# Gregor-Mendel-Institute/SNPmatch

Measured on AMD Instinct MI355X. Metric: accession×SNP comparisons/sec (whole node); achieved HBM GB/s vs peak, higher is better.
Workload: dtype f64

## Files before the change

include/snpmatch_hip.h:

```cpp
#ifndef SNPMATCH_HIP_H
#define SNPMATCH_HIP_H

#include <stdint.h>

#ifdef __cplusplus
extern "C" {
#endif

#define SNPM_OK            0
#define SNPM_ERR_BADARG   -1
#define SNPM_ERR_HIP      -2
#define SNPM_ERR_OOM      -3
#define SNPM_ERR_STATE    -4
#define SNPM_ERR_DOMAIN   -5
#define SNPM_ERR_RCCL     -6

#define SNPM_MODE_EXACT   0
#define SNPM_MODE_STRICT  1
#define SNPM_MODE_FAST    2

typedef struct snpm_ctx   snpm_ctx;
typedef struct snpm_panel snpm_panel;
typedef struct snpm_query snpm_query;
typedef struct snpm_carry snpm_carry;
// ... 108 lines not shown

int snpm_score_dense_host(snpm_ctx *ctx, const int8_t *db, int64_t db_pitch, int64_t n, int64_t n_acc,
                          const double *wei, int skip_hets, double *score, int64_t *ninfo);

int snpm_likelihood(snpm_ctx *ctx, const double *y, const int64_t *n, int64_t m, int64_t len,
                    int truncate, double amin_or_nan, double *lik, double *lrt);
int snpm_likelihood_device(snpm_ctx *ctx, const void *d_y, const void *d_n, int64_t m, int64_t len,
                           int truncate, double amin_or_nan, void *d_lik, void *d_lrt, int *domain_error);

int snpm_binom_identity(snpm_ctx *ctx, const double *x, const int64_t *n, int64_t len, double error_rate,
                        double pthres, int64_t *out, double *sf);
int snpm_binom_sf_host(const double *k, const double *n, int64_t len, double p, double *sf);

int snpm_intersect_sorted(const int64_t *a, int64_t na, const int64_t *b, int64_t nb, int64_t *ia, int64_t *ib,
                          int64_t *n_out);
int snpm_intersect_sorted_search(const int64_t *a, int64_t na, const int64_t *b, int64_t nb, int64_t *ia, int64_t *ib,
                                 int64_t *n_out);
int snpm_panel_segregating(snpm_panel *panel, const int32_t *cols, int64_t ncols, uint8_t *mask);
int snpm_panel_segregating_first(snpm_panel *panel, const int32_t *cols, int64_t ncols, uint8_t *mask, uint8_t *first);
int snpm_query_gather_columns(snpm_query *query, const int32_t *acc_idx, int ncols, uint8_t *codes);
int snpm_query_f1_pairs(snpm_query *query, const int32_t *acc_idx, int n_sel, double *score, int64_t *ninfo);

int snpm_debug_stream_read(snpm_panel *panel, int64_t *bytes_read);
int snpm_profile_enable(snpm_ctx *ctx, int on);
int snpm_profile_reset(snpm_ctx *ctx);
int snpm_profile_read(snpm_ctx *ctx, const char *kernel, int64_t *launches, double *total_ms);

typedef struct snpm_vcf snpm_vcf;
int snpm_vcf_parse(const char *path, int sample_index, snpm_vcf **out);
int snpm_vcf_dims(const snpm_vcf *vcf, int64_t *n_records, int *chr_width, int *gt_width, int *flags, int *n_samples);
int snpm_vcf_fill(const snpm_vcf *vcf, char *chr, int64_t *pos, char *gt, double *pl, int64_t *dp);
int snpm_vcf_fill_u32(const snpm_vcf *vcf, uint32_t *chr, int64_t *pos, uint32_t *gt, double *pl, int64_t *dp, uint8_t *called);
const char *snpm_vcf_sample_name(const snpm_vcf *vcf, int i);
int snpm_vcf_free(snpm_vcf *vcf);

typedef struct snpm_h5 snpm_h5;
int snpm_h5_open(const char *path, snpm_h5 **out);
int snpm_h5_close(snpm_h5 *file);
const char *snpm_h5_last_error(const snpm_h5 *file);
int snpm_h5_list(snpm_h5 *file, const char *group, char *buf, int64_t cap, int64_t *needed);
int snpm_h5_info(snpm_h5 *file, const char *path, const char *attr, int *kind, int *rank, int64_t *dims, int *type_class,
                 int *elem_size, int *is_signed, int64_t *chunk, int *n_attrs);
int snpm_h5_attr_name(snpm_h5 *file, const char *path, int index, char *buf, int64_t cap);
int snpm_h5_read(snpm_h5 *file, const char *path, const char *attr, void *out, int64_t out_bytes);
int snpm_h5_read_rows(snpm_h5 *file, const char *path, const int64_t *row_idx, int64_t file_row0, int64_t nrows, int64_t col0,
                      int64_t ncols, void *out, int64_t out_pitch);
// ... 8 lines not shown
```

snpmatch_amd/_lib.py:

```python
import ctypes as C
import os
import sys

import numpy as np

_HERE = os.path.dirname(os.path.abspath(__file__))
LIB_PATH = os.environ.get("SNPMATCH_HIP_LIB") or os.path.join(_HERE, "libsnpmatch_hip.so")

SNPM_OK = 0
SNPM_ERR_BADARG = -1
SNPM_ERR_HIP = -2
SNPM_ERR_OOM = -3
SNPM_ERR_STATE = -4
SNPM_ERR_DOMAIN = -5
SNPM_ERR_RCCL = -6
GROUP_ID_BYTES = 128
GROUP_LOOPBACK = 1

MODE_EXACT = 0
MODE_STRICT = 1
MODE_FAST = 2

SYMBOLS = [
    "snpm_version", "snpm_hip_build_version", "snpm_build_id", "snpm_device_count", "snpm_init", "snpm_destroy", "snpm_last_error", "snpm_set_stream",
    "snpm_synchronize", "snpm_device_mem_info", "snpm_panel_create", "snpm_panel_create_packed", "snpm_panel_is_packed", "snpm_panel_set_total_accessions", "snpm_panel_row_pitch", "snpm_panel_free", "snpm_panel_info", "snpm_panel_upload_rows", "snpm_panel_load_file", "snpm_panel_load_file_rows", "snpm_panel_load_file_rows_packed", "snpm_pack_rows_host",
    "snpm_panel_upload_wait", "snpm_panel_download_rows", "snpm_panel_fill_synthetic", "snpm_query_create",
    "snpm_query_free", "snpm_query_bind_outputs", "snpm_query_run", "snpm_query_run_device", "snpm_query_error_bound",
    "snpm_query_run_windows", "snpm_query_run_windows_carry", "snpm_score_dense_host", "snpm_likelihood", "snpm_likelihood_device",
    "snpm_binom_identity", "snpm_binom_sf_host", "snpm_intersect_sorted", "snpm_panel_segregating",
    "snpm_query_f1_pairs", "snpm_intersect_sorted_search",
    "snpm_vcf_parse", "snpm_vcf_dims", "snpm_vcf_fill", "snpm_vcf_fill_u32", "snpm_vcf_sample_name", "snpm_vcf_free",
    "snpm_debug_stream_read", "snpm_profile_enable", "snpm_profile_reset", "snpm_profile_read",
    "snpm_panel_fill_synthetic_rows", "snpm_sample_synthetic", "snpm_query_create_device", "snpm_query_last_reeval",
    "snpm_query_last_kernel", "snpm_carry_create", "snpm_carry_reset", "snpm_carry_free", "snpm_carry_set_columns", "snpm_carry_bind_outputs", "snpm_panel_segregating_first", "snpm_query_gather_columns", "snpm_query_run_windows_fast", "snpm_score_batch", "snpm_score_batch_coded", "snpm_batch_configure", "snpm_batch_last_stats", "snpm_genotype_once", "snpm_genotype_once_coded", "snpm_host_alloc", "snpm_host_free",
    "snpm_query_run_carry", "snpm_carry_finish", "snpm_carry_patch", "snpm_carry_device_ptrs", "snpm_carry_error_bound",
    "snpm_group_unique_id", "snpm_group_create_rank", "snpm_group_create_local", "snpm_group_free", "snpm_group_last_error",
    "snpm_group_info", "snpm_group_ctx", "snpm_group_shard", "snpm_group_gather_scores", "snpm_group_gathered_ptrs",
    "snpm_group_transport",
    "snpm_h5_open", "snpm_h5_close", "snpm_h5_last_error", "snpm_h5_list", "snpm_h5_info", "snpm_h5_attr_name", "snpm_h5_read",
    "snpm_h5_read_rows", "snpm_panel_load_h5",
]

_lib = None


class SnpmError(RuntimeError):
    def __init__(self, code, msg):
        RuntimeError.__init__(self, "libsnpmatch_hip error %d: %s" % (code, msg))
        self.code = code
        self.msg = msg


HIP_RUNTIME = "system"


# ... 136 lines not shown
    lib.snpm_host_free.argtypes = [p, p]
    lib.snpm_score_batch.argtypes = [p, i64, p, p, p, ci, i64, ci, ci, p, p, p, p, p]
    lib.snpm_batch_configure.argtypes = [p, ci, ci, dbl]
    lib.snpm_batch_last_stats.argtypes = [p, p]
    lib.snpm_score_dense_host.argtypes = [p, p, i64, i64, i64, p, ci, p, p]
    lib.snpm_likelihood.argtypes = [p, p, p, i64, i64, ci, dbl, p, p]
    lib.snpm_likelihood_device.argtypes = [p, p, p, i64, i64, ci, dbl, p, p, C.POINTER(ci)]
    lib.snpm_binom_identity.argtypes = [p, p, p, i64, dbl, dbl, p, p]
    lib.snpm_binom_sf_host.argtypes = [p, p, i64, dbl, p]
    lib.snpm_intersect_sorted.argtypes = [p, i64, p, i64, p, p, C.POINTER(i64)]
    lib.snpm_panel_segregating.argtypes = [p, p, i64, p]
    lib.snpm_query_f1_pairs.argtypes = [p, p, ci, p, p]
    lib.snpm_panel_segregating_first.argtypes = [p, p, i64, p, p]
    lib.snpm_query_gather_columns.argtypes = [p, p, ci, p]
    lib.snpm_intersect_sorted_search.argtypes = [p, i64, p, i64, p, p, C.POINTER(i64)]
    lib.snpm_vcf_parse.argtypes = [C.c_char_p, ci, pp]
    lib.snpm_vcf_dims.argtypes = [p, C.POINTER(i64), C.POINTER(ci), C.POINTER(ci), C.POINTER(ci), C.POINTER(ci)]
    lib.snpm_vcf_fill.argtypes = [p, p, p, p, p, p]
    lib.snpm_vcf_fill_u32.argtypes = [p, p, p, p, p, p, p]
    lib.snpm_vcf_sample_name.argtypes = [p, ci]
    lib.snpm_vcf_sample_name.restype = C.c_char_p
    lib.snpm_vcf_free.argtypes = [p]
    lib.snpm_debug_stream_read.argtypes = [p, C.POINTER(i64)]
    lib.snpm_profile_enable.argtypes = [p, ci]
    lib.snpm_profile_reset.argtypes = [p]
    lib.snpm_profile_read.argtypes = [p, C.c_char_p, C.POINTER(i64), C.POINTER(dbl)]
    for name in SYMBOLS:
        getattr(lib, name)
    _lib = lib
    return lib


def build_id():
    return load().snpm_build_id().decode()


def check_group(rc, group_handle=None):
    if rc == SNPM_OK:
        return
    msg = load().snpm_group_last_error(group_handle)
    msg = msg.decode("utf-8", "replace") if msg else ""
    if rc == SNPM_ERR_BADARG:
        raise AssertionError(msg)
    if rc == SNPM_ERR_DOMAIN:
        raise AssertionError(msg or "provided y is greater than n")
    if rc == SNPM_ERR_OOM:
# ... 99 lines not shown
```

snpmatch_amd/csrc/snpm_api_launch.hpp:

```cpp
struct FastGeom {
    int bpl, wpb;
    int tile_rows = TILE_ROWS;
    int64_t n_wc, n_colblocks, n_parts, part_rows;
    int64_t n_epochs, n_slots, n_groups;
};

template <int BPL, bool SKIP, bool GATHER, bool NT>
int occupancy_of(int threads)
{
    int nb = 0;
    if (hipOccupancyMaxActiveBlocksPerMultiprocessor(&nb, k_fast<BPL, SKIP, GATHER, NT>, threads, 0) != hipSuccess) nb = 0;
    return nb;
}

int pick_bpl(snpm_ctx *ctx, int64_t n_acc)
{
    (void)n_acc;
    if (ctx->force_bpl == 8 || ctx->force_bpl == 16) return ctx->force_bpl;
    return 4;
}

FastGeom fast_geom(snpm_ctx *ctx, int64_t n_acc, int64_t n, int occ_blocks_hint, int bpl, int tile_rows = TILE_ROWS,
                   int wpb_fixed = 0, int kernel_parts_mult = 1)
{
// ... 41 lines not shown
    n_parts = std::min(n_parts, n_tiles);
    if (ctx->debug_max_parts > 0) n_parts = std::min<int64_t>(n_parts, ctx->debug_max_parts);
    n_parts = std::min<int64_t>(n_parts, 65535);
    g.n_parts = n_parts;
    const int64_t tiles_per_part = (n_tiles + n_parts - 1) / n_parts;
    g.part_rows = tiles_per_part * tile_rows;
    g.n_epochs = std::max<int64_t>(1, (tiles_per_part + EPOCH_TILES - 1) / EPOCH_TILES);
    g.n_slots = g.n_epochs * g.n_parts;
    g.n_groups = (g.n_slots + REDUCE_GROUP - 1) / REDUCE_GROUP;
    return g;
}

template <int BPL, bool SKIP, bool GATHER, bool NT>
int launch_fast_t(snpm_query *q, const FastGeom &g)
{
    snpm_ctx *ctx = q->panel->ctx;
    snpm_panel *p = q->panel;
    dim3 grid((unsigned)g.n_colblocks, (unsigned)g.n_parts);
    dim3 block(WAVE * g.wpb);
    ProfScope ps(ctx, PK_FAST);
    if (BPL == 4 && g.tile_rows == LONG_TILE_ROWS)
        hipLaunchKernelGGL((k_fast<BPL, SKIP, GATHER, NT, false, (BPL == 4 ? LONG_TILE_ROWS : TILE_ROWS)>), grid, block, 0, ctx->stream, p->d,
                           p->pitch, q->d_row_idx, q->row0, q->n, q->d_lut, (double *)ctx->ws_part_score.p, (uint32_t *)ctx->ws_part_miss.p,
                           p->ld, (const int64_t *)nullptr);
    else
        hipLaunchKernelGGL((k_fast<BPL, SKIP, GATHER, NT>), grid, block, 0, ctx->stream, p->d, p->pitch, q->d_row_idx, q->row0,
                           q->n, q->d_lut, (double *)ctx->ws_part_score.p, (uint32_t *)ctx->ws_part_miss.p, p->ld,
                           (const int64_t *)nullptr, (BPL == 4 && g.tile_rows < TILE_ROWS) ? g.tile_rows : 0);
    HIPCHK(ctx, hipGetLastError());
    return SNPM_OK;
}

template <int BPL, bool NT>
int launch_fast_b(snpm_query *q, const FastGeom &g, bool skip, bool gather)
{
    if (skip)
        return gather ? launch_fast_t<BPL, true, true, NT>(q, g) : launch_fast_t<BPL, true, false, NT>(q, g);
    return gather ? launch_fast_t<BPL, false, true, NT>(q, g) : launch_fast_t<BPL, false, false, NT>(q, g);
}

static int q4_waves_per_block(int64_t n_acc)
{
    const int64_t n_wc = (n_acc + 1023) / 1024;
    if (n_wc <= 8) return (int)n_wc;
    int best = 4;
    int64_t best_waves = (n_wc + 3) / 4 * 4;
    for (int w : {7, 8}) {
        const int64_t waves = (n_wc + w - 1) / w * w;
        if (waves <= best_waves) {
            best = w;
// ... 99 lines not shown
```

snpmatch_amd/csrc/snpm_api_oneshot.hpp:

```cpp
int snpm_score_dense_host(snpm_ctx *ctx, const int8_t *db, int64_t db_pitch, int64_t n, int64_t n_acc,
                          const double *wei, int skip_hets, double *score, int64_t *ninfo)
{
    if (!ctx) return SNPM_ERR_BADARG;
    CHECK_ARG(ctx, n >= 0 && n_acc >= 1, "please provide same number of positions for both sample and db");
    CHECK_ARG(ctx, n == 0 || (db != nullptr && wei != nullptr), "NULL input");
    CHECK_ARG(ctx, db_pitch >= n_acc, "db_pitch smaller than n_acc");
    snpm_panel *p = nullptr;
    snpm_query *q = nullptr;
    int rc = snpm_panel_create(ctx, n, n_acc, &p);
    if (rc) return rc;
    rc = snpm_panel_upload_rows(p, 0, n, db, db_pitch);
    if (!rc) rc = snpm_query_create(p, nullptr, 0, n, wei, &q);
    if (!rc) {
        rc = snpm_query_run(q, std::max<int64_t>(n, 1), skip_hets, SNPM_MODE_STRICT, score, ninfo, nullptr);
    }
    std::string keep = ctx->err;
    if (q) snpm_query_free(q);
    (void)snpm_panel_upload_wait(p);
    snpm_panel_free(p);
    if (rc) ctx->err = keep;
    return rc;
}

int snpm_likelihood_device(snpm_ctx *ctx, const void *d_y, const void *d_n, int64_t m, int64_t len, int truncate,
// ... 232 lines not shown
    HIPCHK(ctx, hipStreamSynchronize(st));
    return SNPM_OK;
} SNPM_GUARD(((q && q->panel) ? q->panel->ctx : nullptr))

int snpm_debug_stream_read(snpm_panel *p, int64_t *bytes_read)
{
    CHECK_PANEL(p);
    snpm_ctx *ctx = p->ctx;
    HIPCHK(ctx, hipSetDevice(ctx->device));
    int rc = ensure(ctx, ctx->ws_flags, sizeof(int));
    if (rc) return rc;
    rc = wait_upload(p);
    if (rc) return rc;
    const int64_t n_dwords = p->n_snp * p->pitch / 4;
    const unsigned blocks = (unsigned)std::max<int64_t>(1, std::min<int64_t>((n_dwords + 1023) / 1024, (int64_t)ctx->n_cu * 8));
    hipLaunchKernelGGL(k_calib_read, dim3(blocks), dim3(256), 0, ctx->stream, (const uint32_t *)p->d, n_dwords,
                       (uint32_t *)ctx->ws_flags.p);
    HIPCHK(ctx, hipGetLastError());
    HIPCHK(ctx, hipStreamSynchronize(ctx->stream));
    if (bytes_read) *bytes_read = n_dwords * 4;
    return SNPM_OK;
}

int snpm_host_alloc(snpm_ctx *ctx, int64_t bytes, void **out)
{
    if (!ctx) return SNPM_ERR_BADARG;
    CHECK_ARG(ctx, out != nullptr && bytes >= 0, "bad arguments");
    HIPCHK(ctx, hipSetDevice(ctx->device));
    *out = nullptr;
    hipError_t e = hipHostMalloc(out, (size_t)std::max<int64_t>(bytes, 1), hipHostMallocDefault);
    if (e != hipSuccess) return set_err(ctx, SNPM_ERR_OOM, "hipHostMalloc of %lld bytes failed: %s", (long long)bytes, hipGetErrorString(e));
    return SNPM_OK;
}

int snpm_host_free(snpm_ctx *ctx, void *ptr)
{
    if (!ctx) return SNPM_ERR_BADARG;
    if (ptr && hip_alive()) {
        (void)hipSetDevice(ctx->device);
        (void)hipStreamSynchronize(ctx->copy_stream);
        (void)hipStreamSynchronize(ctx->stream);
        (void)hipHostFree(ptr);
    }
    return SNPM_OK;
}

// ... 1 lines not shown
```

snpmatch_amd/csrc/snpm_api_seg.hpp:

```cpp
struct SegJob {
    snpm_panel *p = nullptr;
    const int64_t *d_row_idx = nullptr;
    int64_t row0 = 0, n_total = 0;
    const double *d_w = nullptr, *d_lut = nullptr;
    const int64_t *seg_off = nullptr;
    int64_t n_seg = 0;
    int64_t chunk = 1000;
    int skip = 0;
    bool certify = true;
    double *d_score = nullptr;
    int64_t *d_ninfo = nullptr;
    int64_t ldo = 0;
    int64_t kmax = 1;
    int cap = 0;
    const int64_t *d_seg_off = nullptr;
};

constexpr int SEG_PAIR_CAP = 32768;

int *seg_pair_count(snpm_ctx *ctx) { return (int *)ctx->ws_pairs.p; }
int32_t *seg_pairs(snpm_ctx *ctx) { return (int32_t *)((char *)ctx->ws_pairs.p + 16); }

template <bool NT>
static int launch_q4_seg(snpm_ctx *ctx, const SegJob &j, dim3 grid, dim3 block, int64_t n_parts, const int64_t *d_desc)
// ... 10 lines not shown
        if (tr == 16) LAUNCH_SEG_TR(S, G, 16);                                                                    \
        else if (tr == 32) LAUNCH_SEG_TR(S, G, 32);                                                               \
        else LAUNCH_SEG_TR(S, G, 64);                                                                             \
    } while (0)
    if (j.skip) {
        if (gather) LAUNCH_SEG(true, true); else LAUNCH_SEG(true, false);
    } else {
        if (gather) LAUNCH_SEG(false, true); else LAUNCH_SEG(false, false);
    }
#undef LAUNCH_SEG_TR
#undef LAUNCH_SEG
    HIPCHK(ctx, hipGetLastError());
    return SNPM_OK;
}

template <int BPL, bool NT>
static int launch_fast_seg(snpm_ctx *ctx, const SegJob &j, dim3 grid, dim3 block, int64_t n_parts, const int64_t *d_desc)
{
    snpm_panel *p = j.p;
    const bool gather = j.d_row_idx != nullptr;
    ProfScope ps(ctx, PK_FAST);
#define LAUNCH_SEG(S, G)                                                                                          \
    hipLaunchKernelGGL((k_fast<BPL, S, G, NT, true>), grid, block, 0, ctx->stream, p->d, p->pitch, j.d_row_idx, j.row0,    \
                       n_parts, j.d_lut, (double *)ctx->ws_part_score.p, (uint32_t *)ctx->ws_part_miss.p, p->ld, d_desc)
    if (j.skip) {
        if (gather) LAUNCH_SEG(true, true); else LAUNCH_SEG(true, false);
    } else {
        if (gather) LAUNCH_SEG(false, true); else LAUNCH_SEG(false, false);
    }
#undef LAUNCH_SEG
    HIPCHK(ctx, hipGetLastError());
    return SNPM_OK;
}

struct SegPlan {
    FastGeom g0;
    int64_t n_parts = 0, tiles_per_part = 0;
    std::vector<int64_t> slot0;
    const int64_t *d_slot0 = nullptr, *d_desc = nullptr;
};

static int seg_plan(snpm_ctx *ctx, SegJob &j, SegPlan &pl)
{
    snpm_panel *p = j.p;
    const int64_t n_seg = j.n_seg;
    const bool q4 = p->packed != 0;
    pl.g0 = q4 ? fast_geom(ctx, p->n_acc, TILE_ROWS, 2, 16, TILE_ROWS, q4_waves_per_block(p->n_acc))
// ... 289 lines not shown
```

snpmatch_amd/csrc/snpm_api_strict.hpp:

```cpp
static inline bool single_accession(const snpm_panel *p) { return p->n_acc_total == 1; }

static int launch_strict_single(snpm_ctx *ctx, const snpm_panel *p, const int64_t *d_row_idx, int64_t row0, const double *d_w,
                                int skip, const int64_t *seg_off, int64_t chunk, int64_t n, int64_t seg0, int64_t n_seg,
                                const int32_t *pairs, const int *count, int cap, int tier, int64_t kmax, dim3 grid,
                                double *out_score, uint32_t *out_miss, int64_t ld)
{
    const bool gather = d_row_idx != nullptr;
#define LAUNCH_SINGLE(S, G)                                                                                          \
    hipLaunchKernelGGL((k_strict_single<S, G>), grid, dim3(SINGLE_THREADS), 0, ctx->stream, p->d, p->kpitch, p->desc,  \
                       d_row_idx, row0, d_w, seg_off, chunk, n, seg0, n_seg, pairs, count, cap, tier, kmax, out_score,  \
                       out_miss, ld)
    if (skip) {
        if (gather) LAUNCH_SINGLE(true, true); else LAUNCH_SINGLE(true, false);
    } else {
        if (gather) LAUNCH_SINGLE(false, true); else LAUNCH_SINGLE(false, false);
    }
#undef LAUNCH_SINGLE
    HIPCHK(ctx, hipGetLastError());
    return SNPM_OK;
}

int launch_strict_dense(snpm_query *q, int skip, const int64_t *d_seg_off, int64_t chunk, int64_t seg0, int64_t n_seg,
                        const int *gate)
{
// ... 113 lines not shown
        dim3 sgrid((unsigned)std::min<int64_t>((total + 255) / 256, (int64_t)ctx->n_cu * 8));
        const bool use_T = !q->transient_panel && q->n >= ctx->acc_major_min_rows && p->dT_state == 1;
        ProfScope ps(ctx, PK_STRICT);
        if (single_accession(p)) {
            q->reeval_path = 2;
            rc = launch_strict_single(ctx, p, q->d_row_idx, q->row0, q->d_w, skip, d_seg_off, chunk, q->n, 0, n_seg, nullptr, d_ncols,
                                      REEVAL_CAP, 1, 0, dim3((unsigned)std::min<int64_t>(n_seg, 65535)),
                                      (double *)ctx->ws_seg_score.p, (uint32_t *)ctx->ws_seg_miss.p, ld);
            if (rc) return rc;
        } else if (use_T) {
            q->reeval_path = 1;
#define LAUNCH_SPARSE_T(S, G)                                                                                      \
    hipLaunchKernelGGL((k_strict_sparse_T<S, G>), sgrid, dim3(256), 0, ctx->stream, p->dT, p->pitchT, q->d_row_idx, \
                       q->row0, q->d_w, d_seg_off, chunk, q->n, n_seg, d_cols, d_ncols, REEVAL_CAP, \
                       (double *)ctx->ws_seg_score.p, (uint32_t *)ctx->ws_seg_miss.p, ld)
            if (skip) {
                if (gather) LAUNCH_SPARSE_T(true, true); else LAUNCH_SPARSE_T(true, false);
            } else {
                if (gather) LAUNCH_SPARSE_T(false, true); else LAUNCH_SPARSE_T(false, false);
            }
#undef LAUNCH_SPARSE_T
        } else {
            q->reeval_path = 2;
#define LAUNCH_SPARSE(S, G)                                                                                        \
    hipLaunchKernelGGL((k_strict_sparse<S, G>), sgrid, dim3(256), 0, ctx->stream, p->d, p->kpitch, p->desc, q->d_row_idx, \
                       q->row0, q->d_w, d_seg_off, chunk, q->n, n_seg, d_cols, d_ncols, REEVAL_CAP, \
                       (double *)ctx->ws_seg_score.p, (uint32_t *)ctx->ws_seg_miss.p, ld)
            if (skip) {
                if (gather) LAUNCH_SPARSE(true, true); else LAUNCH_SPARSE(true, false);
            } else {
                if (gather) LAUNCH_SPARSE(false, true); else LAUNCH_SPARSE(false, false);
            }
#undef LAUNCH_SPARSE
        }
        HIPCHK(ctx, hipGetLastError());
    }
    ProfScope ps(ctx, PK_SCAN);
    if (tail)
        hipLaunchKernelGGL(k_once_tail, dim3(1), dim3(256), 0, ctx->stream, (const double *)ctx->ws_seg_score.p, n_seg, ld, d_ncols,
                           REEVAL_CAP, (double *)ctx->ws_tmp_score.p, d_cols, patch_score, tail->d_ninfo, tail->n_acc, tail->want_lik,
                           tail->state, tail->lik_tmp, tail->out);
    else
        hipLaunchKernelGGL(k_scan_few, dim3(1), dim3(256), 0, ctx->stream, (const double *)ctx->ws_seg_score.p, n_seg, ld,
                           d_ncols, REEVAL_CAP, (double *)ctx->ws_tmp_score.p, carry, d_cols, patch_score);
    HIPCHK(ctx, hipGetLastError());
    return SNPM_OK;
}

// ... 1 lines not shown
```

snpmatch_amd/csrc/snpm_k_fast.hpp:

```cpp
#pragma once

namespace snpm {
typedef uint32_t u32x2 __attribute__((ext_vector_type(2)));
typedef uint32_t u32x4 __attribute__((ext_vector_type(4)));

template <int BPL>
struct LoadT;
template <>
struct LoadT<4> { typedef uint32_t type; };
template <>
struct LoadT<8> { typedef u32x2 type; };
template <>
struct LoadT<16> { typedef u32x4 type; };

__device__ __forceinline__ uint32_t dword_of(const uint32_t &v, int) { return v; }
__device__ __forceinline__ uint32_t dword_of(const u32x2 &v, int k) { return k == 0 ? v.x : v.y; }
__device__ __forceinline__ uint32_t dword_of(const u32x4 &v, int k)
{
    return k == 0 ? v.x : (k == 1 ? v.y : (k == 2 ? v.z : v.w));
}

template <int NDW, bool SKIP, int U>
__device__ __forceinline__ void fast_row(const uint32_t (&x)[NDW], uint32_t group_base, uint32_t roff4,
                                         double (&acc)[NDW * 4], uint32_t (&miss8)[NDW])
// ... 22 lines not shown
#pragma unroll
    for (int e = 0; e < NDW * 4; ++e) acc[e] += w[e];
}

template <int BPL, bool NT>
__device__ __forceinline__ void load_row(const int8_t *p, uint32_t (&x)[BPL / 4])
{
    typedef typename LoadT<BPL>::type load_t;
    load_t v;
    if (NT)
        v = __builtin_nontemporal_load(reinterpret_cast<const load_t *>(p));
    else
        v = *reinterpret_cast<const load_t *>(p);
#pragma unroll
    for (int k = 0; k < BPL / 4; ++k) x[k] = dword_of(v, k);
}

#define SCORE_ROW(U, X, GROUP_BASE, ROFF4, ROFF) fast_row<NDW, SKIP, U>((X), (GROUP_BASE), (ROFF4), acc, miss8)

template <int BPL, bool SKIP, bool GATHER, bool NT, bool SEG = false, int TR = TILE_ROWS>
__global__ void __launch_bounds__(WAVE *MAX_WAVES_PER_BLOCK, (BPL <= 4 ? SNPM_FAST_MIN_WAVES : 1))
k_fast(const int8_t *__restrict__ db, int64_t pitch, const int64_t *__restrict__ row_idx, int64_t row0, int64_t n,
       const double *__restrict__ lut, double *__restrict__ out_score, uint32_t *__restrict__ out_miss, int64_t ld,
       const int64_t *__restrict__ part_desc = nullptr, int tile_rows_rt = 0)
{
    static_assert(BPL == 4 || BPL == 8 || BPL == 16, "int8 panels: 4, 8 or 16 bytes per lane");
    constexpr int NDW = BPL / 4;
    constexpr int EPL = BPL;
    constexpr int G = GATHER ? SNPM_FAST_G_GATHER : SNPM_FAST_G;
    __shared__ __attribute__((aligned(256))) double s_lut[2][TR * 4];
    const int TRR = (tile_rows_rt > 0 && tile_rows_rt <= TR) ? tile_rows_rt : TR;

    const int tid = threadIdx.x;
    const int nthr = blockDim.x;
    const int64_t byte0 = ((int64_t)blockIdx.x * nthr + tid) * BPL;
    const int64_t col0 = byte0;
    const bool lane_on = byte0 < pitch && col0 < ld;
    const int64_t p = SEG ? (int64_t)blockIdx.y + (int64_t)gridDim.y * blockIdx.z : (int64_t)blockIdx.y;
    if (SEG && p >= n) return;
    const int64_t rbase = SEG ? part_desc[3 * p] : 0;
    const int64_t rend = SEG ? part_desc[3 * p + 1] : n;
    const int64_t P = SEG ? 1 : (int64_t)gridDim.y;
    const int64_t T0 = SEG ? 0 : p;
    const int64_t slot0 = SEG ? part_desc[3 * p + 2] : p;
    const int64_t slot_stride = SEG ? 1 : (int64_t)gridDim.y;
    const int64_t n_tiles_total = (rend - rbase + TRR - 1) / TRR;

    double acc[EPL];
    uint32_t miss16[NDW * 2];
    uint32_t miss8[NDW];
#pragma unroll
    for (int i = 0; i < EPL; ++i) acc[i] = 0.0;
#pragma unroll
    for (int i = 0; i < NDW * 2; ++i) miss16[i] = 0;
#pragma unroll
    for (int i = 0; i < NDW; ++i) miss8[i] = 0;

    const uint32_t lane_off = lane_on ? (uint32_t)byte0 : 0u;
    auto row_ptr = [&](int64_t rr) -> const int8_t * {
        const int64_t prow = GATHER ? row_idx[rr] : (row0 + rr);
        const int8_t *rowbase = db + prow * pitch;
        uint32_t off = lane_off;
        asm volatile("" : "+v"(off));
        return rowbase + off;
    };

    auto store_partials = [&](int64_t epoch) {
        if (lane_on) {
            double *os = out_score + (slot0 + epoch * slot_stride) * ld + col0;
            uint32_t *om = out_miss + (slot0 + epoch * slot_stride) * ld + col0;
#pragma unroll
            for (int i = 0; i < EPL; i += 2) *reinterpret_cast<double2 *>(os + i) = make_double2(acc[i], acc[i + 1]);
#pragma unroll
            for (int k = 0; k < NDW; ++k) {
                uint4 m;
                m.x = miss16[2 * k + 0] & 0xffffu;
                m.y = miss16[2 * k + 1] & 0xffffu;
                m.z = miss16[2 * k + 0] >> 16;
                m.w = miss16[2 * k + 1] >> 16;
                *reinterpret_cast<uint4 *>(om + 4 * k) = m;
            }
// ... 114 lines not shown
```

snpmatch_amd/csrc/snpm_k_io.hpp:

```cpp
#pragma once

namespace snpm {
__global__ void k_pack_rows(const int8_t *__restrict__ src, int64_t src_pitch, int64_t nrows, int64_t n_acc,
                            uint8_t *__restrict__ db, int64_t pitch, int64_t desc, int64_t row0, int *__restrict__ bad)
{
    const int64_t row_bytes = pitch + pk_tail_pitch(desc);
    const int64_t i = (int64_t)blockIdx.x * blockDim.x + threadIdx.x;
    if (i >= nrows * row_bytes) return;
    const int64_t r = i / row_bytes, b = i - r * row_bytes;
    uint32_t out = 0;
    int saw = 0;
#pragma unroll
    for (int f = 0; f < 4; ++f) {
        const int64_t a = b * 4 + f;
        int v = -1;
        if (a < n_acc) v = src[r * src_pitch + a];
        saw |= (v > 2);
        out |= (uint32_t)(v < 0 ? 3 : (v & 3)) << (2 * f);
    }
    if (saw) atomicOr(bad, 1);
    db[pk_off(pitch, desc, row0 + r, b)] = (uint8_t)out;
}

__global__ void k_repitch_canon(const int8_t *__restrict__ src, int64_t src_pitch, int64_t nrows, int64_t n_acc,
// ... 121 lines not shown
    }
    wei[3 * r] = w[0];
    wei[3 * r + 1] = w[1];
    wei[3 * r + 2] = w[2];
}

__global__ void __launch_bounds__(256)
k_calib_read(const uint32_t *__restrict__ p, int64_t n_dwords, uint32_t *__restrict__ out)
{
    int64_t i = (int64_t)blockIdx.x * blockDim.x + threadIdx.x;
    const int64_t stride = (int64_t)gridDim.x * blockDim.x;
    uint32_t acc = 0;
    for (; i + 3 * stride < n_dwords; i += 4 * stride) {
        const uint32_t a = __builtin_nontemporal_load(p + i);
        const uint32_t b = __builtin_nontemporal_load(p + i + stride);
        const uint32_t c = __builtin_nontemporal_load(p + i + 2 * stride);
        const uint32_t d = __builtin_nontemporal_load(p + i + 3 * stride);
        acc ^= a ^ b ^ c ^ d;
    }
    for (; i < n_dwords; i += stride) acc ^= __builtin_nontemporal_load(p + i);
    if (acc == 0x9e3779b9u) out[0] = acc;
}

}
```

snpmatch_amd/csrc/snpm_k_strict.hpp:

```cpp
#pragma once

namespace snpm {
template <bool SKIP, bool GATHER>
__global__ void __launch_bounds__(256)
k_strict(const int8_t *__restrict__ db, int64_t pitch, int64_t packed, const int64_t *__restrict__ row_idx, int64_t row0,
         const double *__restrict__ w, const int64_t *__restrict__ seg_off, int64_t chunk, int64_t n, int64_t seg0,
         int64_t n_seg, const int32_t *__restrict__ cols, int64_t ncols, double *__restrict__ out_score,
         uint32_t *__restrict__ out_miss, int64_t ld, const int *__restrict__ gate, int gate_cap)
{
    if (dense_tier_off(gate, gate_cap)) return;
    const int64_t i = (int64_t)blockIdx.y * blockDim.x + threadIdx.x;
    if (i >= ncols) return;
    const int64_t col = cols ? (int64_t)cols[i] : i;
    for (int64_t seg = blockIdx.x; seg < n_seg; seg += gridDim.x) {
    int64_t r0, r1;
    seg_bounds(seg_off, chunk, n, seg_off ? seg : seg0 + seg, r0, r1);
    double a_ref = 0.0, a_het = 0.0, a_alt = 0.0;
    uint32_t miss = 0;
    int64_t r = r0;
    for (; r + 4 <= r1; r += 4) {
        int b[4];
#pragma unroll
        for (int u = 0; u < 4; ++u) {
            const int64_t prow = GATHER ? row_idx[r + u] : (row0 + r + u);
// ... 265 lines not shown
        const int64_t tp = pk_tail_pitch(desc);
        const int64_t byte0 = (int64_t)blockIdx.y * blockDim.x;
        if (tp && byte0 >= pitch) {
            strict4_segments<SKIP, GATHER, true, true>(db + pk_tail_off(desc), tp, row_idx, row0, w, seg_off, chunk, n, seg0, n_seg, ncols,
                                                       out_score, out_miss, ld, c0, s_lut, (uint32_t)pitch);
            return;
        }
        strict4_segments<SKIP, GATHER, true, true>(db, pitch, row_idx, row0, w, seg_off, chunk, n, seg0, n_seg, ncols,
                                                   out_score, out_miss, ld, c0, s_lut);
        return;
    }
    if (c0 >= ncols) return;
    if constexpr (!PACKED && SNPM_STRICT_EXEC) {
        if (*other_codes == 0) {
            strict4_segments<SKIP, GATHER, false, true>(db, pitch, row_idx, row0, w, seg_off, chunk, n, seg0, n_seg, ncols,
                                                        out_score, out_miss, ld, c0, nullptr);
            return;
        }
    }
    strict4_segments<SKIP, GATHER, PACKED, false>(db, pitch, row_idx, row0, w, seg_off, chunk, n, seg0, n_seg, ncols,
                                                  out_score, out_miss, ld, c0, nullptr);
}

template <bool SKIP, bool GATHER>
__global__ void __launch_bounds__(256)
k_strict_sparse(const int8_t *__restrict__ db, int64_t pitch, int64_t packed, const int64_t *__restrict__ row_idx,
                int64_t row0, const double *__restrict__ w, const int64_t *__restrict__ seg_off, int64_t chunk, int64_t n,
                int64_t n_seg, const int32_t *__restrict__ cols, const int *__restrict__ d_ncols, int cap,
                double *__restrict__ out_score, uint32_t *__restrict__ out_miss, int64_t ld)
{
    const int64_t ncols = *d_ncols;
    if (ncols > cap) return;
    for (int64_t id = (int64_t)blockIdx.x * blockDim.x + threadIdx.x; id < n_seg * ncols; id += (int64_t)gridDim.x * blockDim.x) {
    const int64_t seg = id / ncols;
    const int64_t i = id - seg * ncols;
    const int64_t col = cols[i];
    int64_t r0, r1;
    seg_bounds(seg_off, chunk, n, seg, r0, r1);
    double a_ref = 0.0, a_het = 0.0, a_alt = 0.0;
    uint32_t miss = 0;
    constexpr int U = 32;
    int64_t r = r0;
    for (; r + U <= r1; r += U) {
        int b[U];
#pragma unroll
        for (int u = 0; u < U; ++u) {
            const int64_t prow = GATHER ? row_idx[r + u] : (row0 + r + u);
            b[u] = code_at(db, pitch, prow, col, packed);
        }
#pragma unroll
        for (int u = 0; u < U; ++u) {
            const double w0 = w[3 * (r + u) + 0], w1 = w[3 * (r + u) + 1], w2 = w[3 * (r + u) + 2];
            a_ref = add_sel(a_ref, b[u] == 0, w0);
            if (!SKIP) a_het = add_sel(a_het, b[u] == 2, w1);
            a_alt = add_sel(a_alt, b[u] == 1, w2);
            miss += SKIP ? (b[u] < 0 || b[u] == 2) : (b[u] < 0);
        }
    }
    for (; r < r1; ++r) {
        const int64_t prow = GATHER ? row_idx[r] : (row0 + r);
        const int b = code_at(db, pitch, prow, col, packed);
        const double w0 = w[3 * r + 0], w1 = w[3 * r + 1], w2 = w[3 * r + 2];
        a_ref = add_sel(a_ref, b == 0, w0);
        if (!SKIP) a_het = add_sel(a_het, b == 2, w1);
        a_alt = add_sel(a_alt, b == 1, w2);
        miss += SKIP ? (b < 0 || b == 2) : (b < 0);
    }
    out_score[seg * ld + i] = ((0.0 + a_ref) + a_het) + a_alt;
    out_miss[seg * ld + i] = miss;
    }
}

constexpr int PT_ROWS = 256;
constexpr int PT_COLS = 64;
__global__ void __launch_bounds__(256)
k_pack_transpose(const int8_t *__restrict__ db, int64_t pitch, int64_t n_snp, int64_t n_acc,
                 uint8_t *__restrict__ dT, int64_t pitchT, int *__restrict__ bad)
{
    __shared__ uint32_t tile[PT_ROWS][PT_COLS / 4 + 1];
    const int64_t snp0 = (int64_t)blockIdx.x * PT_ROWS;
    const int64_t acc0 = (int64_t)blockIdx.y * PT_COLS;
    const int t = threadIdx.x;
    for (int pass = 0; pass < PT_ROWS / 16; ++pass) {
        const int r = pass * 16 + (t >> 4);
        const int64_t row = snp0 + r;
        uint32_t v = 0xffffffffu;
        if (row < n_snp) v = *reinterpret_cast<const uint32_t *>(db + row * pitch + acc0 + (t & 15) * 4);
        tile[r][t & 15] = v;
    }
    __syncthreads();
    const int c = t & 63, q = t >> 6;
    if (acc0 + c < n_acc) {
// ... 268 lines not shown
```

snpmatch_amd/engine.py:

```python
import atexit
import ctypes as C
import weakref

import numpy as np

from . import _lib
from ._lib import MODE_EXACT, MODE_FAST, MODE_STRICT, check, ptr

_default_ctx = None


class Context(object):
    def __init__(self, device_id=0, _borrowed=None):
        lib = _lib.load()
        if _borrowed is None:
            h = C.c_void_p()
            rc = lib.snpm_init(int(device_id), C.byref(h))
            check(rc, None)
        else:
            h = _borrowed
        self._owns = _borrowed is None
        self.lib = lib
        self.h = h
        self.device_id = int(device_id)
# ... 372 lines not shown

    def fill_synthetic(self, seed, snp0=0, acc0=0, row0=0, nrows=None):
        nrows = self.n_snp - row0 if nrows is None else nrows
        check(self.ctx.lib.snpm_panel_fill_synthetic_rows(self.h, C.c_uint64(int(seed)), int(snp0), int(acc0), int(row0),
                                                          int(nrows)), self.ctx.h)

    def segregating_rows(self, cols):
        cols = np.ascontiguousarray(cols, dtype=np.int32)
        mask = np.zeros(self.n_snp, dtype=np.uint8)
        check(self.ctx.lib.snpm_panel_segregating(self.h, ptr(cols), len(cols), ptr(mask)), self.ctx.h)
        return mask

    def segregating_first(self, cols):
        cols = np.ascontiguousarray(cols, dtype=np.int32)
        mask = np.zeros(self.n_snp, dtype=np.uint8)
        first = np.full(self.n_snp, 0xFF, dtype=np.uint8)
        check(self.ctx.lib.snpm_panel_segregating_first(self.h, ptr(cols), len(cols), ptr(mask), ptr(first)), self.ctx.h)
        return mask, first

    def stream_read(self):
        n = C.c_int64(0)
        check(self.ctx.lib.snpm_debug_stream_read(self.h, C.byref(n)), self.ctx.h)
        return n.value

    def free(self):
        if self.h:
            for q in list(self._queries):
                q.free()
            if self.ctx.h:
                self.ctx.lib.snpm_panel_free(self.h)
            self.h = None

    def __del__(self):
        try:
            self.free()
        except Exception:
            pass


class Query(object):

    def __init__(self, panel, row_idx, wei, row0=0, _device=None):
        self.panel = panel
        ctx = panel.ctx
        if _device is not None:
            d_rows, d_wei, n = _device
# ... 749 lines not shown
```

Measured before the change: 6173 billion.

## Warp-specialize sparse strict reeval with double-buffered LDS tiles and add touch probe

Rewrites k_strict_sparse so that one wave computes while three loader waves prefetch the column codes of the next row tile into a double-buffered shared-memory tile. Several segments are packed into each wave by lane, and the grid is capped at a multiple of the CU count. The aim is to hide the latency of scattered per-column gathers, at the cost of idle lanes when ncols does not divide WAVE and an early exit when ncols exceeds WAVE. Separately, k_fast now checks lane validity against n_acc and clamps inactive lanes to a valid offset, and a debug column-touch timing probe is added.

```diff
diff --git a/include/snpmatch_hip.h b/include/snpmatch_hip.h
--- a/include/snpmatch_hip.h
+++ b/include/snpmatch_hip.h
@@ -154,6 +154,7 @@
 int snpm_query_f1_pairs(snpm_query *query, const int32_t *acc_idx, int n_sel, double *score, int64_t *ninfo);
 
 int snpm_debug_stream_read(snpm_panel *panel, int64_t *bytes_read);
+int snpm_debug_touch_columns(snpm_panel *panel, const int32_t *cols, int k, double *ms, int64_t *touches);
 int snpm_profile_enable(snpm_ctx *ctx, int on);
 int snpm_profile_reset(snpm_ctx *ctx);
 int snpm_profile_read(snpm_ctx *ctx, const char *kernel, int64_t *launches, double *total_ms);
diff --git a/snpmatch_amd/_lib.py b/snpmatch_amd/_lib.py
--- a/snpmatch_amd/_lib.py
+++ b/snpmatch_amd/_lib.py
@@ -30,7 +30,7 @@
     "snpm_binom_identity", "snpm_binom_sf_host", "snpm_intersect_sorted", "snpm_panel_segregating",
     "snpm_query_f1_pairs", "snpm_intersect_sorted_search",
     "snpm_vcf_parse", "snpm_vcf_dims", "snpm_vcf_fill", "snpm_vcf_fill_u32", "snpm_vcf_sample_name", "snpm_vcf_free",
-    "snpm_debug_stream_read", "snpm_profile_enable", "snpm_profile_reset", "snpm_profile_read",
+    "snpm_debug_stream_read", "snpm_debug_touch_columns", "snpm_profile_enable", "snpm_profile_reset", "snpm_profile_read",
     "snpm_panel_fill_synthetic_rows", "snpm_sample_synthetic", "snpm_query_create_device", "snpm_query_last_reeval",
     "snpm_query_last_kernel", "snpm_carry_create", "snpm_carry_reset", "snpm_carry_free", "snpm_carry_set_columns", "snpm_carry_bind_outputs", "snpm_panel_segregating_first", "snpm_query_gather_columns", "snpm_query_run_windows_fast", "snpm_score_batch", "snpm_score_batch_coded", "snpm_batch_configure", "snpm_batch_last_stats", "snpm_genotype_once", "snpm_genotype_once_coded", "snpm_host_alloc", "snpm_host_free",
     "snpm_query_run_carry", "snpm_carry_finish", "snpm_carry_patch", "snpm_carry_device_ptrs", "snpm_carry_error_bound",
@@ -213,6 +213,7 @@
     lib.snpm_vcf_sample_name.restype = C.c_char_p
     lib.snpm_vcf_free.argtypes = [p]
     lib.snpm_debug_stream_read.argtypes = [p, C.POINTER(i64)]
+    lib.snpm_debug_touch_columns.argtypes = [p, C.POINTER(C.c_int32), C.c_int, C.POINTER(C.c_double), C.POINTER(i64)]
     lib.snpm_profile_enable.argtypes = [p, ci]
     lib.snpm_profile_reset.argtypes = [p]
     lib.snpm_profile_read.argtypes = [p, C.c_char_p, C.POINTER(i64), C.POINTER(dbl)]
diff --git a/snpmatch_amd/csrc/snpm_api_launch.hpp b/snpmatch_amd/csrc/snpm_api_launch.hpp
--- a/snpmatch_amd/csrc/snpm_api_launch.hpp
+++ b/snpmatch_amd/csrc/snpm_api_launch.hpp
@@ -87,10 +87,10 @@
     if (BPL == 4 && g.tile_rows == LONG_TILE_ROWS)
         hipLaunchKernelGGL((k_fast<BPL, SKIP, GATHER, NT, false, (BPL == 4 ? LONG_TILE_ROWS : TILE_ROWS)>), grid, block, 0, ctx->stream, p->d,
                            p->pitch, q->d_row_idx, q->row0, q->n, q->d_lut, (double *)ctx->ws_part_score.p, (uint32_t *)ctx->ws_part_miss.p,
-                           p->ld, (const int64_t *)nullptr);
+                           p->ld, p->n_acc, (const int64_t *)nullptr);
     else
         hipLaunchKernelGGL((k_fast<BPL, SKIP, GATHER, NT>), grid, block, 0, ctx->stream, p->d, p->pitch, q->d_row_idx, q->row0,
-                           q->n, q->d_lut, (double *)ctx->ws_part_score.p, (uint32_t *)ctx->ws_part_miss.p, p->ld,
+                           q->n, q->d_lut, (double *)ctx->ws_part_score.p, (uint32_t *)ctx->ws_part_miss.p, p->ld, p->n_acc,
                            (const int64_t *)nullptr, (BPL == 4 && g.tile_rows < TILE_ROWS) ? g.tile_rows : 0);
     HIPCHK(ctx, hipGetLastError());
     return SNPM_OK;
diff --git a/snpmatch_amd/csrc/snpm_api_oneshot.hpp b/snpmatch_amd/csrc/snpm_api_oneshot.hpp
--- a/snpmatch_amd/csrc/snpm_api_oneshot.hpp
+++ b/snpmatch_amd/csrc/snpm_api_oneshot.hpp
@@ -278,6 +278,44 @@
     return SNPM_OK;
 }
 
+int snpm_debug_touch_columns(snpm_panel *p, const int32_t *cols, int k, double *ms, int64_t *touches)
+{
+    CHECK_PANEL(p);
+    snpm_ctx *ctx = p->ctx;
+    CHECK_ARG(ctx, !p->packed, "the touch probe reads int8 panels");
+    CHECK_ARG(ctx, cols != nullptr && k >= 1 && k <= 1024, "cols: 1..1024 accession columns");
+    for (int j = 0; j < k; ++j) CHECK_ARG(ctx, cols[j] >= 0 && cols[j] < p->n_acc, "column out of range");
+    HIPCHK(ctx, hipSetDevice(ctx->device));
+    int rc = ensure(ctx, ctx->ws_flags, sizeof(int));
+    if (rc) return rc;
+    rc = wait_upload(p);
+    if (rc) return rc;
+    int32_t *d_cols = nullptr;
+    HIPCHK(ctx, hipMalloc(&d_cols, (size_t)k * sizeof(int32_t)));
+    hipEvent_t e0 = nullptr, e1 = nullptr;
+    hipError_t err = hipMemcpyAsync(d_cols, cols, (size_t)k * sizeof(int32_t), hipMemcpyHostToDevice, ctx->stream);
+    if (err == hipSuccess) err = hipEventCreate(&e0);
+    if (err == hipSuccess) err = hipEventCreate(&e1);
+    const unsigned blocks = (unsigned)ctx->n_cu * 8;
+    for (int it = 0; it < 2 && err == hipSuccess; ++it) {
+        if (it == 1) err = hipEventRecord(e0, ctx->stream);
+        hipLaunchKernelGGL(k_touch_cols, dim3(blocks), dim3(256), 0, ctx->stream, p->d, p->pitch, p->n_snp, d_cols, k,
+                           (uint32_t *)ctx->ws_flags.p);
+        if (err == hipSuccess) err = hipGetLastError();
+    }
+    if (err == hipSuccess) err = hipEventRecord(e1, ctx->stream);
+    if (err == hipSuccess) err = hipEventSynchronize(e1);
+    float t = 0.0f;
+    if (err == hipSuccess) err = hipEventElapsedTime(&t, e0, e1);
+    if (e0) (void)hipEventDestroy(e0);
+    if (e1) (void)hipEventDestroy(e1);
+    (void)hipFree(d_cols);
+    HIPCHK(ctx, err);
+    if (ms) *ms = t;
+    if (touches) *touches = p->n_snp * (int64_t)k;
+    return SNPM_OK;
+}
+
 int snpm_host_alloc(snpm_ctx *ctx, int64_t bytes, void **out)
 {
     if (!ctx) return SNPM_ERR_BADARG;
diff --git a/snpmatch_amd/csrc/snpm_api_seg.hpp b/snpmatch_amd/csrc/snpm_api_seg.hpp
--- a/snpmatch_amd/csrc/snpm_api_seg.hpp
+++ b/snpmatch_amd/csrc/snpm_api_seg.hpp
@@ -56,7 +56,7 @@
     ProfScope ps(ctx, PK_FAST);
 #define LAUNCH_SEG(S, G)                                                                                          \
     hipLaunchKernelGGL((k_fast<BPL, S, G, NT, true>), grid, block, 0, ctx->stream, p->d, p->pitch, j.d_row_idx, j.row0,    \
-                       n_parts, j.d_lut, (double *)ctx->ws_part_score.p, (uint32_t *)ctx->ws_part_miss.p, p->ld, d_desc)
+                       n_parts, j.d_lut, (double *)ctx->ws_part_score.p, (uint32_t *)ctx->ws_part_miss.p, p->ld, p->n_acc, d_desc)
     if (j.skip) {
         if (gather) LAUNCH_SEG(true, true); else LAUNCH_SEG(true, false);
     } else {
diff --git a/snpmatch_amd/csrc/snpm_api_strict.hpp b/snpmatch_amd/csrc/snpm_api_strict.hpp
--- a/snpmatch_amd/csrc/snpm_api_strict.hpp
+++ b/snpmatch_amd/csrc/snpm_api_strict.hpp
@@ -159,8 +159,9 @@
 #undef LAUNCH_SPARSE_T
         } else {
             q->reeval_path = 2;
+            const dim3 rgrid((unsigned)std::min<int64_t>(n_seg, (int64_t)ctx->n_cu * 6));
 #define LAUNCH_SPARSE(S, G)                                                                                        \
-    hipLaunchKernelGGL((k_strict_sparse<S, G>), sgrid, dim3(256), 0, ctx->stream, p->d, p->kpitch, p->desc, q->d_row_idx, \
+    hipLaunchKernelGGL((k_strict_sparse<S, G>), rgrid, dim3(SPARSE_THREADS), 0, ctx->stream, p->d, p->kpitch, p->desc, q->d_row_idx, \
                        q->row0, q->d_w, d_seg_off, chunk, q->n, n_seg, d_cols, d_ncols, REEVAL_CAP, \
                        (double *)ctx->ws_seg_score.p, (uint32_t *)ctx->ws_seg_miss.p, ld)
             if (skip) {
diff --git a/snpmatch_amd/csrc/snpm_k_fast.hpp b/snpmatch_amd/csrc/snpm_k_fast.hpp
--- a/snpmatch_amd/csrc/snpm_k_fast.hpp
+++ b/snpmatch_amd/csrc/snpm_k_fast.hpp
@@ -68,7 +68,7 @@
 __global__ void __launch_bounds__(WAVE *MAX_WAVES_PER_BLOCK, (BPL <= 4 ? SNPM_FAST_MIN_WAVES : 1))
 k_fast(const int8_t *__restrict__ db, int64_t pitch, const int64_t *__restrict__ row_idx, int64_t row0, int64_t n,
        const double *__restrict__ lut, double *__restrict__ out_score, uint32_t *__restrict__ out_miss, int64_t ld,
-       const int64_t *__restrict__ part_desc = nullptr, int tile_rows_rt = 0)
+       int64_t n_acc, const int64_t *__restrict__ part_desc = nullptr, int tile_rows_rt = 0)
 {
     static_assert(BPL == 4 || BPL == 8 || BPL == 16, "int8 panels: 4, 8 or 16 bytes per lane");
     constexpr int NDW = BPL / 4;
@@ -81,7 +81,7 @@
     const int nthr = blockDim.x;
     const int64_t byte0 = ((int64_t)blockIdx.x * nthr + tid) * BPL;
     const int64_t col0 = byte0;
-    const bool lane_on = byte0 < pitch && col0 < ld;
+    const bool lane_on = col0 < n_acc;
     const int64_t p = SEG ? (int64_t)blockIdx.y + (int64_t)gridDim.y * blockIdx.z : (int64_t)blockIdx.y;
     if (SEG && p >= n) return;
     const int64_t rbase = SEG ? part_desc[3 * p] : 0;
@@ -102,7 +102,7 @@
 #pragma unroll
     for (int i = 0; i < NDW; ++i) miss8[i] = 0;
 
-    const uint32_t lane_off = lane_on ? (uint32_t)byte0 : 0u;
+    const uint32_t lane_off = lane_on ? (uint32_t)byte0 : (uint32_t)((n_acc - 1) / BPL * BPL);
     auto row_ptr = [&](int64_t rr) -> const int8_t * {
         const int64_t prow = GATHER ? row_idx[rr] : (row0 + rr);
         const int8_t *rowbase = db + prow * pitch;
diff --git a/snpmatch_amd/csrc/snpm_k_io.hpp b/snpmatch_amd/csrc/snpm_k_io.hpp
--- a/snpmatch_amd/csrc/snpm_k_io.hpp
+++ b/snpmatch_amd/csrc/snpm_k_io.hpp
@@ -167,4 +167,30 @@
     if (acc == 0x9e3779b9u) out[0] = acc;
 }
 
+__global__ void __launch_bounds__(256)
+k_touch_cols(const int8_t *__restrict__ db, int64_t pitch, int64_t n_rows, const int32_t *__restrict__ cols, int k,
+             uint32_t *__restrict__ out)
+{
+    const int64_t total = n_rows * k;
+    const int64_t stride = (int64_t)gridDim.x * blockDim.x;
+    int64_t i = (int64_t)blockIdx.x * blockDim.x + threadIdx.x;
+    uint32_t acc = 0;
+    for (; i + 7 * stride < total; i += 8 * stride) {
+        int8_t b[8];
+#pragma unroll
+        for (int u = 0; u < 8; ++u) {
+            const int64_t id = i + u * stride;
+            const int64_t row = id / k;
+            b[u] = db[row * pitch + cols[id - row * k]];
+        }
+#pragma unroll
+        for (int u = 0; u < 8; ++u) acc ^= (uint32_t)(uint8_t)b[u] << (u & 3) * 8;
+    }
+    for (; i < total; i += stride) {
+        const int64_t row = i / k;
+        acc ^= (uint32_t)(uint8_t)db[row * pitch + cols[i - row * k]];
+    }
+    if (acc == 0x9e3779b9u) out[0] = acc;
 }
+
+}
diff --git a/snpmatch_amd/csrc/snpm_k_strict.hpp b/snpmatch_amd/csrc/snpm_k_strict.hpp
--- a/snpmatch_amd/csrc/snpm_k_strict.hpp
+++ b/snpmatch_amd/csrc/snpm_k_strict.hpp
@@ -311,52 +311,99 @@
                                                   out_score, out_miss, ld, c0, nullptr);
 }
 
+constexpr int SPARSE_LOADERS = 3;
+constexpr int SPARSE_TILE_ROWS = 64 * SPARSE_LOADERS;
+constexpr int SPARSE_THREADS = WAVE * (SPARSE_LOADERS + 1);
 template <bool SKIP, bool GATHER>
-__global__ void __launch_bounds__(256)
+__global__ void __launch_bounds__(SPARSE_THREADS)
 k_strict_sparse(const int8_t *__restrict__ db, int64_t pitch, int64_t packed, const int64_t *__restrict__ row_idx,
                 int64_t row0, const double *__restrict__ w, const int64_t *__restrict__ seg_off, int64_t chunk, int64_t n,
                 int64_t n_seg, const int32_t *__restrict__ cols, const int *__restrict__ d_ncols, int cap,
                 double *__restrict__ out_score, uint32_t *__restrict__ out_miss, int64_t ld)
 {
-    const int64_t ncols = *d_ncols;
-    if (ncols > cap) return;
-    for (int64_t id = (int64_t)blockIdx.x * blockDim.x + threadIdx.x; id < n_seg * ncols; id += (int64_t)gridDim.x * blockDim.x) {
-    const int64_t seg = id / ncols;
-    const int64_t i = id - seg * ncols;
-    const int64_t col = cols[i];
-    int64_t r0, r1;
-    seg_bounds(seg_off, chunk, n, seg, r0, r1);
-    double a_ref = 0.0, a_het = 0.0, a_alt = 0.0;
-    uint32_t miss = 0;
-    constexpr int U = 32;
-    int64_t r = r0;
-    for (; r + U <= r1; r += U) {
-        int b[U];
-#pragma unroll
-        for (int u = 0; u < U; ++u) {
-            const int64_t prow = GATHER ? row_idx[r + u] : (row0 + r + u);
-            b[u] = code_at(db, pitch, prow, col, packed);
-        }
-#pragma unroll
-        for (int u = 0; u < U; ++u) {
-            const double w0 = w[3 * (r + u) + 0], w1 = w[3 * (r + u) + 1], w2 = w[3 * (r + u) + 2];
-            a_ref = add_sel(a_ref, b[u] == 0, w0);
-            if (!SKIP) a_het = add_sel(a_het, b[u] == 2, w1);
-            a_alt = add_sel(a_alt, b[u] == 1, w2);
-            miss += SKIP ? (b[u] < 0 || b[u] == 2) : (b[u] < 0);
-        }
-    }
-    for (; r < r1; ++r) {
-        const int64_t prow = GATHER ? row_idx[r] : (row0 + r);
-        const int b = code_at(db, pitch, prow, col, packed);
-        const double w0 = w[3 * r + 0], w1 = w[3 * r + 1], w2 = w[3 * r + 2];
-        a_ref = add_sel(a_ref, b == 0, w0);
-        if (!SKIP) a_het = add_sel(a_het, b == 2, w1);
-        a_alt = add_sel(a_alt, b == 1, w2);
-        miss += SKIP ? (b < 0 || b == 2) : (b < 0);
-    }
-    out_score[seg * ld + i] = ((0.0 + a_ref) + a_het) + a_alt;
-    out_miss[seg * ld + i] = miss;
+    __shared__ int8_t s_code[2][SPARSE_TILE_ROWS * WAVE];
+    const int ncols = *d_ncols;
+    if (ncols < 1 || ncols > cap || ncols > WAVE) return;
+    const int spb = WAVE / ncols;
+    const int c = threadIdx.x & (WAVE - 1);
+    const int wv = threadIdx.x / WAVE;
+    const int sl = c / ncols, ci = c - sl * ncols;
+    const bool chain_on = c < spb * ncols;
+    const int64_t col = chain_on ? (int64_t)cols[ci] : 0;
+    for (int64_t sb = blockIdx.x; sb * spb < n_seg; sb += gridDim.x) {
+        const int64_t seg = sb * spb + sl;
+        int64_t r0 = 0, r1 = 0;
+        if (chain_on && seg < n_seg) seg_bounds(seg_off, chunk, n, seg, r0, r1);
+        const int64_t len = r1 - r0;
+        int64_t len_max = len;
+#pragma unroll
+        for (int d = WAVE / 2; d >= 1; d >>= 1) {
+            const int64_t o = __shfl_xor(len_max, d);
+            len_max = o > len_max ? o : len_max;
+        }
+        const int64_t n_tiles = (len_max + SPARSE_TILE_ROWS - 1) / SPARSE_TILE_ROWS;
+        auto load_tile = [&](int64_t t) {
+            if (wv == 0 || len == 0) return;
+            int8_t *dst = &s_code[t & 1][0];
+            const int64_t rt = t * SPARSE_TILE_ROWS + (int64_t)(wv - 1) * 64;
+#pragma unroll
+            for (int u0 = 0; u0 < 64; u0 += 16) {
+                int b[16];
+#pragma unroll
+                for (int u = 0; u < 16; ++u) {
+                    int64_t rr = rt + u0 + u;
+                    rr = r0 + (rr < len ? rr : len - 1);
+                    const int64_t prow = GATHER ? row_idx[rr] : (row0 + rr);
+                    b[u] = code_at(db, pitch, prow, col, packed);
+                }
+#pragma unroll
+                for (int u = 0; u < 16; ++u) dst[((wv - 1) * 64 + u0 + u) * WAVE + c] = (int8_t)b[u];
+            }
+        };
+        double a_ref = 0.0, a_het = 0.0, a_alt = 0.0;
+        uint32_t miss = 0;
+        if (n_tiles > 0) load_tile(0);
+        __syncthreads();
+        for (int64_t t = 0; t < n_tiles; ++t) {
+            if (t + 1 < n_tiles) load_tile(t + 1);
+            if (wv == 0 && len > t * SPARSE_TILE_ROWS) {
+                const int8_t *src = &s_code[t & 1][0];
+                const int64_t rt = t * SPARSE_TILE_ROWS;
+                const int rows = (int)((len - rt < SPARSE_TILE_ROWS) ? (len - rt) : SPARSE_TILE_ROWS);
+                const double *wr = w + 3 * (r0 + rt);
+                int r = 0;
+                for (; r + 8 <= rows; r += 8) {
+                    int b[8];
+                    double w0[8], w1[8], w2[8];
+#pragma unroll
+                    for (int u = 0; u < 8; ++u) {
+                        b[u] = src[(r + u) * WAVE + c];
+                        w0[u] = wr[3 * (r + u) + 0];
+                        w1[u] = wr[3 * (r + u) + 1];
+                        w2[u] = wr[3 * (r + u) + 2];
+                    }
+#pragma unroll
+                    for (int u = 0; u < 8; ++u) {
+                        a_ref = add_sel(a_ref, b[u] == 0, w0[u]);
+                        if (!SKIP) a_het = add_sel(a_het, b[u] == 2, w1[u]);
+                        a_alt = add_sel(a_alt, b[u] == 1, w2[u]);
+                        miss += SKIP ? (b[u] < 0 || b[u] == 2) : (b[u] < 0);
+                    }
+                }
+                for (; r < rows; ++r) {
+                    const int b = src[r * WAVE + c];
+                    a_ref = add_sel(a_ref, b == 0, wr[3 * r + 0]);
+                    if (!SKIP) a_het = add_sel(a_het, b == 2, wr[3 * r + 1]);
+                    a_alt = add_sel(a_alt, b == 1, wr[3 * r + 2]);
+                    miss += SKIP ? (b < 0 || b == 2) : (b < 0);
+                }
+            }
+            __syncthreads();
+        }
+        if (wv == 0 && chain_on && seg < n_seg) {
+            out_score[seg * ld + ci] = ((0.0 + a_ref) + a_het) + a_alt;
+            out_miss[seg * ld + ci] = miss;
+        }
     }
 }
 
diff --git a/snpmatch_amd/engine.py b/snpmatch_amd/engine.py
--- a/snpmatch_amd/engine.py
+++ b/snpmatch_amd/engine.py
@@ -418,6 +418,13 @@
         n = C.c_int64(0)
         check(self.ctx.lib.snpm_debug_stream_read(self.h, C.byref(n)), self.ctx.h)
         return n.value
+
+    def touch_columns(self, cols):
+        cols = np.ascontiguousarray(cols, dtype=np.int32)
+        ms, n = C.c_double(0.0), C.c_int64(0)
+        check(self.ctx.lib.snpm_debug_touch_columns(self.h, cols.ctypes.data_as(C.POINTER(C.c_int32)), len(cols), C.byref(ms),
+                                                     C.byref(n)), self.ctx.h)
+        return ms.value, n.value
 
     def free(self):
         if self.h:
```

New measurement: 6239 billion, median of 6. 1.01x the previous value.
